# y00njaekim/CMU-11785-IDL-1.58bit-ASR

Measured on AMD Instinct MI355X. Metric: mel-frames/sec (Conformer-S 1.58-bit train step), higher is better.
Workload: dtype fp32; 1 GPU; conformer-s-1.58bit-train-step; global_batch=32, execution=hip-graph, per_gpu_batch=32, frames=1000, d_model=144, blocks=16, d_ff=576, heads=4, vocab=5004, parallelism=dp1, passes=teacher 2-bit + student 1-bit + SP, conv_pointwise=fp32 (reference)

## Files before the change

cmu-11785-idl-1.58bit-asr_amd/csrc/capi.hip:

```cpp
#include <float.h>

#include <algorithm>
#include <vector>

#include "../../include/onebit_hip.h"
#include "ob_launch.h"
#include <stdint.h>

using namespace ob;

namespace {

constexpr int kAbiVersion = 4;

inline hipStream_t as_stream(void* s) { return reinterpret_cast<hipStream_t>(s); }

inline bool aligned4(const void* p) { return (reinterpret_cast<uintptr_t>(p) & 3) == 0; }
inline bool misaligned8(const void* p) { return (reinterpret_cast<uintptr_t>(p) & 7) != 0; }

inline int check_bits(int bits) { return (bits == 1 || bits == 2) ? OB_OK : OB_ERR_BITWIDTH; }

inline int launched() {
  const hipError_t e = hipGetLastError();
  return e == hipSuccess ? OB_OK : OB_ERR_HIP;
// ... 2029 lines not shown
                          void* table, int64_t slot2, int64_t slot1, void* stream) {
  if (rows < 0 || !layernorm_supported(d) || !(p_drop >= 0.0f && p_drop < 1.0f))
    return OB_ERR_SHAPE;
  if (rows > 0 && (!dy || !y1 || !mean2 || !rstd2 || !x || !mean1 || !rstd1 || !dx || !ws))
    return OB_ERR_NULL;
  if (dy2 && p_drop > 0.0f && !rng) return OB_ERR_NULL;
  if (ws_bytes < 2 * layernorm_bwd_workspace(rows, d)) return OB_ERR_WORKSPACE;
  if (!aligned4(dy) || !aligned4(y1) || !aligned4(gres) || !aligned4(x) || !aligned4(dx) ||
      !aligned4(dy2) || !aligned4(g1) || !aligned4(g2) || !aligned4(lens) || ((uintptr_t)ws & 15))
    return OB_ERR_ALIGN;
  if (dy2 && lens && (T < 1 || T > 0x7fffffff || rows % T)) return OB_ERR_SHAPE;
  LnGradScale gsc{dy2, rscale, p_drop, rng, (uint64_t)rng_offset, lens, (int)T};
  LnParamEntry* tab = static_cast<LnParamEntry*>(table);
  const LnDefer f2{tab && slot2 >= 0 ? tab : nullptr, (int)slot2};
  const LnDefer f1{tab && slot1 >= 0 ? tab : nullptr, (int)slot1};
  launch_layernorm_bwd_pair(dy, y1, g2, mean2, rstd2, gres, x, g1, mean1, rstd1, rows, d, dx, dg2,
                            db2, dg1, db1, ws, as_stream(stream), dy2 ? &gsc : nullptr, &f2, &f1);
  return launched();
}

int ob_layernorm_bwd_defer(const float* dy, const float* x, const float* gamma, const float* mean,
                           const float* rstd, int64_t rows, int64_t d, const float* dres,
                           float* dx, float* dgamma, float* dbeta, void* ws, size_t ws_bytes,
                           float* dy2, float rscale, float p_drop, const uint64_t* rng,
                           int64_t rng_offset, const int32_t* lens, int64_t T, void* table,
                           int64_t slot, void* stream) {
  if (table && slot < 0) return OB_ERR_SHAPE;
  if (rows < 0 || !layernorm_supported(d)) return OB_ERR_SHAPE;
  if (rows > 0 && (!dy || !x || !mean || !rstd || !dx)) return OB_ERR_NULL;
  if ((dgamma || dbeta) && !ws) return OB_ERR_NULL;
  if ((dgamma || dbeta) && ws_bytes < layernorm_bwd_workspace(rows, d)) return OB_ERR_WORKSPACE;
  if (!aligned4(dy) || !aligned4(x) || !aligned4(dx) || !aligned4(dres) || !aligned4(dy2) ||
      !aligned4(lens))
    return OB_ERR_ALIGN;
  if (dy2) {
    if (!(p_drop >= 0.0f && p_drop < 1.0f)) return OB_ERR_SHAPE;
    if (lens && (T < 1 || T > 0x7fffffff || rows % T)) return OB_ERR_SHAPE;
    if (p_drop > 0.0f && !rng) return OB_ERR_NULL;
  }
  LnGradScale gs{dy2, rscale, p_drop, rng, (uint64_t)rng_offset,
                 reinterpret_cast<const int*>(lens), (int)T};
  const LnDefer df{static_cast<LnParamEntry*>(table), (int)slot};
  launch_layernorm_bwd(dy, x, gamma, mean, rstd, rows, d, dres, dx, dgamma, dbeta, ws,
                       as_stream(stream), &gs, &df);
  return launched();
}

namespace {
int relattn_check(int64_t Bt, int64_t P, int64_t T, int64_t H, int64_t d, float p_drop) {
  if (Bt < 1 || P < 1 || Bt % P != 0 || H < 1 || !relattn_supported(T, d)) return OB_ERR_SHAPE;
  if (Bt > 65535 || H > 65535 || !(p_drop >= 0.0f && p_drop < 1.0f)) return OB_ERR_SHAPE;
  return OB_OK;
}
}

int ob_relattn_fwd(const float* q, const float* k, const float* v, const float* pos,
                   const float* u, const float* vb, const int32_t* lens, int64_t Bt, int64_t P,
                   int64_t T, int64_t H, int64_t d, float p_drop, const int64_t* rng,
                   int64_t rng_offset, float* saved, float* probs, float* ctx, void* stream) {
  if (int st = relattn_check(Bt, P, T, H, d, p_drop)) return st;
  if (!q || !k || !v || !pos || !u || !vb || !lens || !ctx || (p_drop > 0.0f && !rng))
    return OB_ERR_NULL;
  if (((uintptr_t)saved & 15) || ((uintptr_t)probs & 15)) return OB_ERR_ALIGN;
  launch_relattn_fwd(q, k, v, pos, u, vb, lens, Bt, P, T, H, d, p_drop,
                     reinterpret_cast<const uint64_t*>(rng), (uint64_t)rng_offset, saved, probs,
                     ctx, as_stream(stream));
  return launched();
}

int64_t ob_relattn_saved_elems(int64_t Bt, int64_t T, int64_t H, int64_t d) {
  if (Bt < 1 || H < 1 || !relattn_supported(T, d)) return 0;
  return relattn_saved_elems(Bt, T, H, d);
}

size_t ob_relattn_bwd_workspace(int64_t Bt, int64_t T, int64_t H, int64_t d) {
  if (Bt < 1 || H < 1 || !relattn_supported(T, d)) return 0;
  return align_up(relattn_bwd_workspace(Bt, T, H, d));
}

int ob_relattn_set_bwd_mode(int mode) { return relattn_set_flash(mode); }

int ob_tgemm_set_colloop(int on) { return tgemm_set_colloop(on); }

int64_t ob_relattn_probs_elems(int64_t Bt, int64_t T, int64_t H) {
  if (Bt < 1 || H < 1 || T < 1) return 0;
  return relattn_probs_elems(Bt, T, H);
}

int ob_relattn_bwd(const float* dctx, const float* ctx, const float* q, const float* k,
                   const float* v, const float* pos, const float* u, const float* vb,
                   const int32_t* lens, int64_t Bt, int64_t P, int64_t T, int64_t H, int64_t d,
                   float p_drop, const int64_t* rng, int64_t rng_offset, const float* saved,
                   int64_t saved_elems, float* dq, float* dk, float* dv, float* dpos, float* du,
                   float* dvb, void* ws, size_t ws_bytes, void* stream) {
  if (int st = relattn_check(Bt, P, T, H, d, p_drop)) return st;
  if (!dctx || !ctx || !q || !k || !v || !pos || !u || !vb || !lens || !saved || !dq || !dk ||
      !dv || !dpos || !du || !dvb || !ws)
    return OB_ERR_NULL;
  if (saved_elems != relattn_saved_elems(Bt, T, H, d)) return OB_ERR_SHAPE;
  (void)rng;
  (void)rng_offset;
  if ((uintptr_t)saved & 15) return OB_ERR_ALIGN;
  if (ws_bytes < ob_relattn_bwd_workspace(Bt, T, H, d)) return OB_ERR_WORKSPACE;
  launch_relattn_bwd(dctx, ctx, q, k, v, pos, u, vb, lens, Bt, P, T, H, d, p_drop, saved, dq, dk,
                     dv, dpos, du, dvb, ws, as_stream(stream));
  return launched();
}

int ob_decattn_supported(int64_t Lq, int64_t Lk, int64_t dh) {
  return decattn_supported(Lq, Lk, dh) ? 1 : 0;
}

static int decattn_check(int64_t B, int64_t H, int64_t Lq, int64_t Lk, int64_t dh, int64_t sq,
                         int64_t sk, int64_t sv, float p_drop) {
  if (B < 0 || H < 1 || !decattn_supported(Lq, Lk, dh) || !(p_drop >= 0.0f && p_drop < 1.0f))
    return OB_ERR_SHAPE;
  if (sq < H * dh || sk < H * dh || sv < H * dh) return OB_ERR_SHAPE;
  if (B * H * Lq > INT32_MAX) return OB_ERR_SHAPE;
  return OB_OK;
}

int ob_decattn_fwd(const float* q, int64_t sq, const float* k, int64_t sk, const float* v,
                   int64_t sv, const uint8_t* kmask, int64_t causal, int64_t B, int64_t H,
                   int64_t Lq, int64_t Lk, int64_t dh, float p_drop, const int64_t* rng,
                   int64_t rng_offset, float* probs, float* ctx, void* stream) {
  if (int st = decattn_check(B, H, Lq, Lk, dh, sq, sk, sv, p_drop)) return st;
  if (B > 0 && (!q || !k || !v || !probs || !ctx || (p_drop > 0.0f && !rng))) return OB_ERR_NULL;
  if (!aligned4(q) || !aligned4(k) || !aligned4(v) || !aligned4(probs) ||
      (reinterpret_cast<uintptr_t>(ctx) & 15))
    return OB_ERR_ALIGN;
  launch_decattn_fwd(q, sq, k, sk, v, sv, kmask, causal ? 1 : 0, B, H, Lq, Lk, dh, p_drop,
                     reinterpret_cast<const uint64_t*>(rng), (uint64_t)rng_offset, probs, ctx,
                     as_stream(stream));
  return launched();
}

int ob_decattn_fwd_grouped(const float* q, int64_t sq, const float* k, int64_t sk, const float* v,
                           int64_t sv, const uint8_t* kmask, int64_t causal, int64_t B,
                           int64_t kv_group, int64_t H, int64_t Lq, int64_t Lk, int64_t dh,
                           float* ctx, void* stream) {
  if (kv_group < 1 || B < 0 || (B > 0 && kv_group > INT32_MAX / B)) return OB_ERR_SHAPE;
  if (int st = decattn_check(B * kv_group, H, Lq, Lk, dh, sq, sk, sv, 0.0f)) return st;
  if (B > 0 && (!q || !k || !v || !ctx)) return OB_ERR_NULL;
  if (!aligned4(q) || !aligned4(k) || !aligned4(v) || (reinterpret_cast<uintptr_t>(ctx) & 15))
    return OB_ERR_ALIGN;
  launch_decattn_fwd_grouped(q, sq, k, sk, v, sv, kmask, causal ? 1 : 0, B, kv_group, H, Lq, Lk,
                             dh, ctx, as_stream(stream));
  return launched();
}

int ob_decattn_bwd(const float* dctx, const float* ctx, const float* q, int64_t sq, const float* k,
                   int64_t sk, const float* v, int64_t sv, int64_t B, int64_t H, int64_t Lq, int64_t Lk,
                   int64_t dh, float p_drop, float* probs, float* dq, int64_t gq, float* dk,
                   int64_t gk, float* dv, int64_t gv, void* stream) {
  if (int st = decattn_check(B, H, Lq, Lk, dh, sq, sk, sv, p_drop)) return st;
  if (gq < H * dh || gk < H * dh || gv < H * dh) return OB_ERR_SHAPE;
  if (B > 0 && (!dctx || !ctx || !q || !k || !v || !probs || !dq || !dk || !dv)) return OB_ERR_NULL;
  if (!aligned4(ctx) || !aligned4(dctx) || !aligned4(q) || !aligned4(k) || !aligned4(v) || !aligned4(probs) ||
      !aligned4(dq) || !aligned4(dk) || !aligned4(dv))
    return OB_ERR_ALIGN;
  launch_decattn_bwd(dctx, ctx, q, sq, k, sk, v, sv, B, H, Lq, Lk, dh, p_drop, probs, dq, gq, dk, gk,
                     dv, gv, as_stream(stream));
  return launched();
}

int ob_relattn_dropout_mask(int64_t n, int64_t row_len, float p_drop, const int64_t* rng,
// ... 46 lines not shown
```

cmu-11785-idl-1.58bit-asr_amd/csrc/dgemm.hip:

```cpp
#include <algorithm>
#include <cstdlib>

#include "ob_drop.h"
#include "ob_fp.h"
#include "ob_launch.h"
#include "ob_mma.h"

namespace ob {

namespace {

constexpr size_t kLdsCU = 160 * 1024;

__host__ __device__ inline int dg_kpad(int K, int nch) { return nch > 0 ? 32 * nch : (K + 31) & ~31; }
__host__ __device__ inline size_t dg_lds_bytes(int nt, int kpad) {
  return (size_t)16 * nt * 3 * (kpad + 8) * sizeof(uint16_t);
}

template <int NT, int NCH, int WAVES, bool TRANS, bool RES = false>
__global__ __launch_bounds__(64 * WAVES, 2) void dgemm_kernel(
    const float* __restrict__ A, int64_t M, int K, const float* __restrict__ W, int N, int n_ct,
    int n16, int rgroups, const float* __restrict__ bias, float* __restrict__ C,
    const float* __restrict__ R, DropCfg dc, const uint64_t* __restrict__ rng, uint64_t rng_off) {
  constexpr int kThr = 64 * WAVES, BN = 16 * NT;
  extern __shared__ __attribute__((aligned(16))) char smem[];
  __bf16* bimg = reinterpret_cast<__bf16*>(smem);
  const int kpad = dg_kpad(K, NCH);
  const int stride = kpad + 8;
  const int cpitch = 3 * stride;

  const int L = xcd_logical(blockIdx.x, gridDim.x);
  const int ct = L % n_ct;
  const int rg = L / n_ct;
  const int n0 = ct * BN;
  const int s0 = (int)((int64_t)rg * n16 / rgroups), s1 = (int)((int64_t)(rg + 1) * n16 / rgroups);
  const int lane = threadIdx.x & 63;
  const int wave = threadIdx.x >> 6;
  const int r = lane & 15;
  const int g = lane >> 4;
  const int kg = 8 * g;

  const int kq = kpad >> 2;
  const int units = BN * kq;
  auto unit_cols = [&](int u, int& c, int& k4) {
    if constexpr (TRANS) {
      k4 = u / BN;
      c = u - k4 * BN;
    } else {
      c = u / kq;
      k4 = u - c * kq;
    }
  };
  auto unit_load = [&](int u) -> f32x4 {
    u = u < units ? u : units - 1;
    int c, k4;
    unit_cols(u, c, k4);
    const int n = n0 + c < N ? n0 + c : N - 1;
    const int kk = 4 * k4 < K - 4 ? 4 * k4 : K - 4;
    if constexpr (TRANS) {
      const float* p = W + (int64_t)kk * N + n;
      return f32x4{p[0], p[N], p[2 * N], p[3 * N]};
    } else {
      return *reinterpret_cast<const f32x4*>(W + (int64_t)n * K + kk);
    }
  };
  auto unit_store = [&](int u, f32x4 v) {
    if (u >= units) return;
    int c, k4;
    unit_cols(u, c, k4);
    const bool ok = 4 * k4 < K && n0 + c < N;
    const f32x4 x = ok ? v : f32x4{0.f, 0.f, 0.f, 0.f};
    bf16x4 h, m, l;
    split3x4(x, h, m, l);
    __bf16* col = bimg + c * cpitch + 4 * k4;
    *reinterpret_cast<bf16x4*>(col) = h;
    *reinterpret_cast<bf16x4*>(col + stride) = m;
    *reinterpret_cast<bf16x4*>(col + 2 * stride) = l;
  };
  auto arow_of = [&](int j) {
    const int64_t row = (int64_t)16 * j + r < M ? (int64_t)16 * j + r : M - 1;
    return A + row * (int64_t)K;
  };
  const int j0 = s0 + wave;

// ... 167 lines not shown
    u = u < kUnits ? u : kUnits - 1;
    int c, k4;
    unit_cols(u, c, k4);
    const bool ok = ch * kKc + 4 * k4 < K && c < N;
    const f32x4 x = ok ? v : f32x4{0.f, 0.f, 0.f, 0.f};
    bf16x4 h, m, l;
    split3x4(x, h, m, l);
    __bf16* col = img + buf * kBuf + c * kCpitch + 4 * k4;
    *reinterpret_cast<bf16x4*>(col) = h;
    *reinterpret_cast<bf16x4*>(col + kKcStride) = m;
    *reinterpret_cast<bf16x4*>(col + 2 * kKcStride) = l;
  };
  constexpr int kWin = 4;
  f32x4 abuf[kWin][2];
  auto load_a = [&](int st, f32x4& x0, f32x4& x1) { load8(arow, 32 * st + kg, K, x0, x1); };

  f32x4 wv[kUpt];
#pragma unroll
  for (int i = 0; i < kUpt; ++i) wv[i] = unit_load(0, threadIdx.x + i * kThr);
#pragma unroll
  for (int w = 0; w < kWin; ++w) load_a(w, abuf[w][0], abuf[w][1]);
  __builtin_amdgcn_sched_barrier(0);
#pragma unroll
  for (int i = 0; i < kUpt; ++i) unit_store(0, 0, threadIdx.x + i * kThr, wv[i]);
  __syncthreads();

  f32x4 acc[NT];
#pragma unroll
  for (int t = 0; t < NT; ++t) acc[t] = f32x4{0.f, 0.f, 0.f, 0.f};
  for (int ch0 = 0; ch0 < nck; ch0 += 2) {
#pragma unroll
    for (int cc = 0; cc < 2; ++cc) {
      const int ch = ch0 + cc;
      if (ch >= nck) break;
      const int chn = ch + 1 < nck ? ch + 1 : ch;
#pragma unroll
      for (int i = 0; i < kUpt; ++i) wv[i] = unit_load(chn, threadIdx.x + i * kThr);
      const __bf16* brow = img + cc * kBuf + r * kCpitch + kg;
#pragma unroll
      for (int hs = 0; hs < 2; ++hs) {
        const int st = 2 * ch + hs, slot = 2 * cc + hs;
        const f32x4 x0 = abuf[slot][0], x1 = abuf[slot][1];
        load_a(st + kWin, abuf[slot][0], abuf[slot][1]);
        __builtin_amdgcn_sched_barrier(0);
        constexpr int kG = NT < 3 ? NT : 3;
#pragma unroll
        for (int t0 = 0; t0 < NT; t0 += kG) {
          bf16x8 b[kG][3];
#pragma unroll
          for (int t = 0; t < kG; ++t)
#pragma unroll
            for (int q = 0; q < 3; ++q)
              if (t0 + t < NT)
                b[t][q] = *reinterpret_cast<const bf16x8*>(brow + (t0 + t) * 16 * kCpitch +
                                                            q * kKcStride + 32 * hs);
          __builtin_amdgcn_sched_barrier(0);
          bf16x8 a[3];
          split3x8(x0, x1, a[0], a[1], a[2]);
#pragma unroll
          for (int p = 0; p < 6; ++p)
#pragma unroll
            for (int t = 0; t < kG; ++t)
              if (t0 + t < NT) acc[t0 + t] = mfma_bf16(a[kProdA[p]], b[t][kProdB[p]], acc[t0 + t]);
        }
      }
#pragma unroll
      for (int i = 0; i < kUpt; ++i) unit_store(chn, cc ^ 1, threadIdx.x + i * kThr, wv[i]);
      __syncthreads();
    }
  }
#pragma unroll
  for (int t = 0; t < NT; ++t) {
    const int col = 16 * t + r;
    if (col >= N) continue;
    const float bc = bias ? bias[col] : 0.0f;
#pragma unroll
    for (int reg = 0; reg < 4; ++reg) {
      const int64_t orow = m0 + 4 * g + reg;
      if (orow < M) C[orow * N + col] = acc[t][reg] + bc;
    }
  }
}

struct DgCfg {
  int nt, waves;
};

DgCfg pick_cfg(int64_t N, int64_t K) {
  const int kpad = dg_kpad((int)K, 0);
  const bool k_special = kpad == 160 || kpad == 288;
  static const int cands[] = {9, 6, 3, 2, 1};
  for (int pass = 0; pass < 2; ++pass)
    for (int nt : cands) {
      if (pass == 0 && N % (16 * nt) != 0) continue;
      if (16 * nt > ((N + 15) & ~int64_t(15))) continue;
      const bool inst = kpad == 160 ? (nt == 9 || nt == 6 || nt == 3)
                        : kpad == 288 ? (nt == 3 || nt == 2 || nt == 1)
                                      : (nt == 3 || nt == 1);
      if (!inst && k_special) continue;
      if (!k_special && !(nt == 3 || nt == 1)) continue;
      const size_t lds = dg_lds_bytes(nt, kpad);
      int waves = lds <= kLdsCU / 2 ? 4 : lds <= kLdsCU ? 8 : 0;
      if (waves) return DgCfg{nt, waves};
    }
  return DgCfg{0, 0};
}

}

static bool dense_kc_shape(int64_t K, int64_t N) {
  return N >= 4 && N <= 144 && N % 4 == 0 && K >= 4 && K % 4 == 0 && K <= (1 << 20) &&
         pick_cfg(N, K).nt == 0;
}

bool dense_gemm_supported(int64_t K, int64_t N) {
  return (K >= 4 && N >= 4 && K % 4 == 0 && N % 4 == 0 && K <= (1 << 20) && N <= (1 << 20) &&
          pick_cfg(N, K).nt > 0) ||
         dense_kc_shape(K, N);
}

bool launch_dense_gemm(const float* A, int64_t M, int64_t K, const float* W, int trans,
                       const float* bias, int64_t N, float* C, hipStream_t s,
                       const DenseEpi* epi) {
  if (!dense_gemm_supported(K, N)) return false;
  if (M == 0) return true;
  if (dense_kc_shape(K, N)) {
    if (epi && epi->R) return false;
    constexpr int kW = 8;
    const dim3 grid((unsigned)ceil_div(M, 16 * kW));
    const size_t lds = dgkc_lds_bytes(9);
    if (trans)
      hipLaunchKernelGGL((dgemm_kc_kernel<9, kW, true>), grid, dim3(64 * kW), lds, s, A, M, (int)K,
                         W, (int)N, bias, C);
    else
      hipLaunchKernelGGL((dgemm_kc_kernel<9, kW, false>), grid, dim3(64 * kW), lds, s, A, M,
                         (int)K, W, (int)N, bias, C);
    return true;
  }
  const DgCfg cfg = pick_cfg(N, K);
  const int kpad = dg_kpad((int)K, 0);
  const size_t lds = dg_lds_bytes(cfg.nt, kpad);
  const int n_ct = (int)ceil_div(N, 16 * cfg.nt);
  const int n16 = (int)ceil_div(M, 16);
  const int per_cu = (int)std::min<size_t>(kLdsCU / lds, (size_t)(8 / cfg.waves));
  int rgroups = 256 * per_cu / n_ct;
  rgroups = std::min<int64_t>(rgroups, ceil_div(n16, cfg.waves));
  if (rgroups < 1) rgroups = 1;
  const dim3 grid((unsigned)(rgroups * n_ct));
  const int nch = kpad == 160 ? 5 : kpad == 288 ? 9 : 0;
  const float* R = epi ? epi->R : nullptr;
  const DropCfg dc = make_drop(R ? epi->p_drop : 0.0f);
  const uint64_t* rng = R ? epi->rng : nullptr;
  const uint64_t rng_off = R ? epi->rng_off : 0;
#define OB_DG(NT, NCH, WV)                                                                       \
  if (cfg.nt == NT && nch == NCH && cfg.waves == WV) {                                           \
    if (trans)                                                                                   \
      hipLaunchKernelGGL((dgemm_kernel<NT, NCH, WV, true>), grid, dim3(64 * WV), lds, s, A, M,    \
                         (int)K, W, (int)N, n_ct, n16, rgroups, bias, C, nullptr, dc,    \
                         nullptr, 0);                                                            \
    else                                                                                         \
      hipLaunchKernelGGL((dgemm_kernel<NT, NCH, WV, false>), grid, dim3(64 * WV), lds, s, A, M,   \
                         (int)K, W, (int)N, n_ct, n16, rgroups, bias, C, nullptr, dc,    \
                         nullptr, 0);                                                            \
    return true;                                                                                 \
  }
#define OB_DG2(NT, NCH) OB_DG(NT, NCH, 4) OB_DG(NT, NCH, 8)
  if (R && !trans && cfg.nt == 9 && nch == 5) {
#define OB_DGR(WV)                                                                               \
    if (cfg.waves == WV) {                                                                       \
      hipLaunchKernelGGL((dgemm_kernel<9, 5, WV, false, true>), grid, dim3(64 * WV), lds, s, A,   \
                         M, (int)K, W, (int)N, n_ct, n16, rgroups, bias, C, R, dc, rng,         \
                         rng_off);                                                               \
      return true;                                                                               \
    }
    OB_DGR(4)
    OB_DGR(8)
#undef OB_DGR
  }
  if (R) {
    DenseEpi none{nullptr, 0.0f, nullptr, 0};
    if (!launch_dense_gemm(A, M, K, W, trans, bias, N, C, s, &none)) return false;
    launch_residual_drop_fwd(R, C, M, N, 1.0f, epi->p_drop, rng, rng_off, nullptr, 0, C, s);
    return true;
  }
  OB_DG2(9, 5)
  OB_DG2(6, 5)
  OB_DG2(3, 5)
  OB_DG2(3, 9)
  OB_DG2(2, 9)
  OB_DG2(1, 9)
  OB_DG2(3, 0)
  OB_DG2(1, 0)
#undef OB_DG2
#undef OB_DG
  return false;
}

}
```

cmu-11785-idl-1.58bit-asr_amd/csrc/ob_launch.h:

```cpp
#pragma once

#include <hip/hip_runtime.h>
#include <stddef.h>
#include <stdint.h>

#include "../../include/onebit_hip.h"

namespace ob {

inline int64_t ceil_div(int64_t a, int64_t b) { return (a + b - 1) / b; }

void launch_quant_pack(const float* W, const float* alpha, int alpha_raw, int bits,
                       const int* bits_dev, int64_t N, int64_t K, uint32_t* codes,
                       uint32_t* codes_t, hipStream_t s);
int64_t quant_pack_item_blocks(int64_t N, int64_t K);
int64_t quant_pack_item_blocks16(int64_t N, int64_t K);
void launch_quant_pack_group(const ob_pack_item* items_dev, int n_items, int64_t total_blocks,
                             hipStream_t s);
void launch_quant_dequant(const float* W, const float* alpha, int alpha_raw, int bits, int64_t n,
                          float* W_hat, hipStream_t s);

int64_t ste_reduce_blocks(int64_t total);
void launch_ste_reduce(const float* part, int chunks, int64_t nk, const float* part_db,
                       int64_t n_db, const float* W, const float* alpha, int alpha_raw, int bits,
// ... 119 lines not shown
  const float* W;
  const float* alpha;
  int alpha_raw;
  int bits;
  const int* bits_dev;
  const int* pass_bits;
  float* apart;
};
void launch_dw_partial(const float* dY, const float* X, int64_t M, int64_t N, int64_t K,
                       const DwPlan& p, float* part, float* part_db, uint32_t* ticket,
                       hipStream_t s, const DwAlpha* al = nullptr);
void launch_dw_partial_group(const float* const* dY, int G, const float* X, int64_t M,
                             int64_t N, int64_t K, const DwPlan& p, float* const* part,
                             float* const* part_db, const DwAlpha* al, hipStream_t s);
void launch_dw_finish(const float* part, int chunks, int64_t nk, const float* part_db,
                      int64_t n_db, const float* W, const float* alpha, int alpha_raw,
                      const float* apart, int n_apart, float* dW, float* db, float* dalpha,
                      hipStream_t s);

struct DwFinish {
  const float* part;
  int chunks;
  int64_t nk;
  const float* part_db;
  int64_t n_db;
  const float* W;
  const float* alpha;
  int alpha_raw;
  const float* apart;
  int n_apart;
  float* dW;
  float* db;
  float* dalpha;
};
constexpr int kMaxDwGroup = 3;
void launch_dw_finish_group(const DwFinish* a, int n, hipStream_t s);

struct DwFinishEntry {
  DwFinish f;
  int64_t start;
};
int64_t dw_finish_blocks(const DwFinish& a);
void launch_dw_table_entry(DwFinishEntry* table, int slot, const DwFinishEntry& ent, hipStream_t s);
void launch_dw_finish_table(const DwFinishEntry* table, int n, int64_t total_blocks, hipStream_t s);
void launch_dw_partial_group_defer(const float* const* dY, int G, const float* X, int64_t M,
                                   int64_t N, int64_t K, const DwPlan& p, float* const* part,
                                   float* const* part_db, const DwAlpha* al,
                                   DwFinishEntry* table, int slot, const DwFinishEntry* ent,
                                   hipStream_t s);

struct DwgDesc {
  const float* dY;
  const float* X;
  const float* W;
  const float* alpha;
  const int* pass_bits;
  float* dW;
  float* db;
  float* dalpha;
  int64_t work0;
  int N, K, Mp, P, alpha_raw, bits;
  int spp;
  int tiles_k;
  int tiles;
  int tile0;
};
constexpr int kDwgTile = 144;
int dwg_blocks(int64_t total_steps);
size_t dwg_slot_bytes();
void launch_dw_grouped(const DwgDesc* host_descs, int G, int64_t total_steps, int blocks,
                       DwgDesc* table, float* slots, float* talpha, uint32_t* tickets,
                       int total_tiles, hipStream_t s);

bool dense_gemm_supported(int64_t K, int64_t N);
struct DenseEpi {
  const float* R;
  float p_drop;
  const uint64_t* rng;
  uint64_t rng_off;
};
bool launch_dense_gemm(const float* A, int64_t M, int64_t K, const float* W, int trans,
                       const float* bias, int64_t N, float* C, hipStream_t s,
                       const DenseEpi* epi = nullptr);

bool ternary_gemm_i8_supported(int64_t K, int64_t N);
void launch_silu_monotone_check(uint32_t lo, uint32_t hi, uint32_t* bad, hipStream_t s);
size_t act_absmax_workspace(int P);
void launch_act_absmax(const float* X, int P, int64_t n_per_pass, float* amax, void* ws,
                       hipStream_t s);
void launch_act_dequant(const float* X, int P, int64_t n_per_pass, const float* amax, float* Xd,
                        hipStream_t s);
bool launch_ternary_gemm_i8(const float* A, int P, int64_t M, int64_t K, const uint32_t* codes,
                            const uint32_t* codes1, const int* pass_bits, int64_t N,
                            const float* alpha, int alpha_raw, const float* amax,
                            const float* bias, float* C, hipStream_t s);

void launch_ctc_greedy(const float* logits, const int64_t* lens, int64_t B, int64_t T, int64_t V,
                       int blank, int* ids, int* out, int* out_len, hipStream_t s);

struct CtcBeamLm {
  const void* table;
  int64_t slots;
  int max_probe, order;
  double unk_logp;
  int bos, eos;
  double lm_weight, ins_bonus;
  double *ctc, *lm, *total;
};
size_t ctc_beam_workspace(int64_t B, int64_t T, int64_t V, int beam, int top_k);
void launch_ctc_beam(const float* logits, const int64_t* lens, int64_t B, int64_t T, int64_t V,
                     int blank, int beam, int top_k, int stages, void* ws, int* hyp, int* hyp_len,
                     int* n_hyp, double* score, int nbest, const CtcBeamLm* lm, hipStream_t s);

bool seq_logprob_supported(int64_t d, int64_t V);
size_t seq_logprob_workspace(int64_t R, int64_t d, int64_t V);
void launch_seq_logprob(const float* hidden, int64_t R, int64_t d, const float* weight,
                        const float* bias, int64_t V, const int* target, void* ws, float* lp,
                        hipStream_t s);
void launch_rescore_prepare(const int* hyp, const int* hyp_len, const int* n_hyp, int64_t B,
                            int64_t N, int64_t T, int64_t Lc, int bos, int eos, int pad,
                            int64_t* tgt_inp, int* target, uint8_t* tgt_pad, uint8_t* ok,
                            hipStream_t s);
void launch_rescore_select(const float* lp, const int* hyp, const int* hyp_len, const int* n_hyp,
                           const double* ctc, const double* lm, const uint8_t* ok, int64_t B,
                           int64_t N, int64_t T, int64_t Lc, double ctc_weight, double lm_weight,
                           int* out, int* out_len, int* best_k, double* att, double* total,
                           uint8_t* rescored, hipStream_t s);

constexpr int kSeqTopkMaxBanned = 8;
struct AttdecState {
  double* score;
  int* len;
  uint8_t* fin;
  int64_t* tok;
  uint8_t* skip;
};
bool attdec_supported(int64_t N, int64_t d, int64_t H, int64_t Lk, int64_t L);
void launch_decattn_step(const float* qkv, int64_t sq, float* cache, const int* anc,
                         const uint8_t* skip, int64_t R, int64_t H, int64_t dh, int64_t L,
                         int64_t t, float* ctx, hipStream_t s);
size_t seq_topk_workspace(int64_t R, int64_t d, int64_t V, int64_t K);
void launch_seq_topk(const float* hidden, int64_t R, int64_t d, const float* weight,
                     const float* bias, int64_t V, const int* banned, int n_banned,
                     const uint8_t* skip, int64_t K, void* ws, double* lse, float* topv,
                     int* topi, hipStream_t s);
void launch_attdec_init(const uint8_t* kmask, int64_t B, int64_t N, int64_t Lk, int64_t L, int bos,
                        const AttdecState& st, int* anc, hipStream_t s);
constexpr int kStepBeam = 0, kStepJoint = 1, kStepFused = 2;
void launch_attdec_step(int mode, const double* lse, const float* topv, const int* topi,
                        const double* cpsi, double w, const double* lmsc, double lw, int64_t B,
                        int64_t N, int64_t K, int64_t L, int64_t t, int eos, int pad,
                        const double* norm, const int* anc_in, int* anc_out,
                        const AttdecState& st, double* att, double* ctc, double* lm, int* link,
                        int* tr_parent, int* tr_token, double* tr_score, hipStream_t s);
void launch_attdec_finalize(const int* tr_parent, const int* tr_token, const AttdecState& st,
                            int64_t B, int64_t N, int64_t L, int eos, int* hyp, int* hyp_len,
                            int* n_hyp, double* score, uint8_t* finished, hipStream_t s);

bool ctc_prefix_supported(int64_t N, int64_t K, int64_t Tp);
size_t ctc_prefix_workspace(int64_t B, int64_t N, int64_t K, int64_t Tp);
void launch_ctc_frame_lse(const float* logits, const int64_t* lens, int64_t B, int64_t Tp,
                          int64_t V, double* flse, hipStream_t s);
void launch_ctc_prefix_step(const float* logits, const double* flse, const int64_t* lens,
                            const int* topi, const int64_t* tok, const int* len, const int* link,
                            const uint8_t* skip, int64_t B, int64_t N, int64_t K, int64_t Tp,
                            int64_t V, int blank, int eos, const double* st_in, double* st_out,
// ... 202 lines not shown
```

cmu-11785-idl-1.58bit-asr_amd/onebit_asr/_lib.py:

```python
from __future__ import annotations

import ctypes
import os
from pathlib import Path

import torch

LIB_NAME = "libonebit_hip.so"
LIB_PATH = Path(os.environ.get("ONEBIT_HIP_LIB") or Path(__file__).with_name(LIB_NAME))

OB_OK = 0
OB_ERR_SHAPE = -2
OB_ERR_BITWIDTH = -3

_c_f = ctypes.c_void_p
_i64 = ctypes.c_int64
_int = ctypes.c_int
_sz = ctypes.c_size_t
_f32 = ctypes.c_float
_f64 = ctypes.c_double

SIGNATURES = {
    "ob_abi_version": (_int, []),
    "ob_source_digest": (ctypes.c_char_p, []),
# ... 171 lines not shown
    "ob_nbest_edit_distance": (_int, [_c_f, _c_f, _c_f, _c_f, _c_f, _i64, _i64, _i64, _i64, _c_f,
                                      _sz, _c_f, _c_f, _c_f, _c_f]),
    "ob_mbr_select": (_int, [_c_f, _c_f, _c_f, _c_f, _c_f, _f64, _i64, _i64, _i64, _c_f, _c_f,
                             _c_f, _c_f, _c_f, _c_f]),
    "ob_fbank_num_frames": (_i64, [_i64]),
    "ob_frontend_table_floats": (_i64, [_int]),
    "ob_frontend_table_fill": (_int, [_c_f, _int]),
    "ob_frontend_fwd": (_int, [_c_f, _i64, _c_f, _i64, _i64, _c_f, _int, _c_f, _c_f, _c_f, _int,
                               _int, _int, _int, _c_f, _i64, _c_f, _c_f]),
    "ob_layernorm_fwd": (_int, [_c_f, _c_f, _c_f, _i64, _i64, _f32, _c_f, _c_f, _c_f, _c_f]),
    "ob_layernorm_fwd_pair": (_int, [_c_f, _c_f, _c_f, _c_f, _c_f, _i64, _i64, _f32, _f32, _c_f,
                                     _c_f, _c_f, _c_f, _c_f, _c_f, _c_f]),
    "ob_layernorm_fwd_amax_workspace": (_sz, [_i64]),
    "ob_layernorm_fwd_amax": (_int, [_c_f, _c_f, _c_f, _i64, _i64, _f32, _c_f, _c_f, _c_f, _i64,
                                     _c_f, _c_f, _sz, _c_f]),
    "ob_layernorm_fwd_i8": (_int, [_c_f, _c_f, _c_f, _i64, _i64, _f32, _i64, _c_f, _c_f, _c_f,
                                   _sz, _c_f]),
    "ob_layernorm_bwd_defer": (
        _int, [_c_f, _c_f, _c_f, _c_f, _c_f, _i64, _i64, _c_f, _c_f, _c_f, _c_f, _c_f, _sz, _c_f,
               _f32, _f32, _c_f, _i64, _c_f, _i64, _c_f, _i64, _c_f]),
    "ob_layernorm_bwd_pair_workspace": (_sz, [_i64, _i64]),
    "ob_layernorm_bwd_pair": (
        _int, [_c_f, _c_f, _c_f, _c_f, _c_f, _c_f, _c_f, _c_f, _c_f, _c_f, _i64, _i64, _c_f, _c_f,
               _c_f, _c_f, _c_f, _c_f, _sz, _c_f, _f32, _f32, _c_f, _i64, _c_f, _i64, _c_f, _i64,
               _i64, _c_f]),
    "ob_ln_param_entry_bytes": (_sz, []),
    "ob_ln_param_table": (_int, [_c_f, _i64, _i64, _c_f]),
    "ob_dw_finish_entry_bytes": (_sz, []),
    "ob_bitlinear_bwd_dw_passes_defer": (
        _int, [_c_f, _c_f, _i64, _i64, _i64, _i64, _c_f, _c_f, _int, _c_f, _c_f, _c_f, _c_f, _c_f,
               _sz, _c_f, _i64, _i64, _c_f, _c_f]),
    "ob_bitlinear_bwd_dw_passes_group_defer": (
        _int, [_i64, _c_f, _c_f, _i64, _i64, _i64, _i64, _c_f, _c_f, _int, _c_f, _c_f, _c_f, _c_f,
               _c_f, _sz, _c_f, _i64, _i64, _c_f, _c_f]),
    "ob_dw_finish_table": (_int, [_c_f, _i64, _i64, _c_f]),
    "ob_dw_grouped_supported": (_int, [_i64, _i64]),
    "ob_dw_grouped_workspace": (_sz, [_c_f, _i64]),
    "ob_dw_grouped_tickets": (_sz, [_c_f, _i64]),
    "ob_dw_grouped": (_int, [_c_f, _i64, _c_f, _sz, _c_f, _sz, _c_f]),
    "ob_dense_dw_defer": (_int, [_c_f, _c_f, _i64, _i64, _i64, _c_f, _c_f, _c_f, _sz, _c_f, _i64,
                                 _i64, _c_f, _c_f]),
    "ob_layernorm_bwd_workspace": (_sz, [_i64, _i64]),
    "ob_layernorm_bwd": (
        _int, [_c_f, _c_f, _c_f, _c_f, _c_f, _i64, _i64, _c_f, _c_f, _c_f, _c_f, _sz, _c_f]),
    "ob_layernorm_bwd_res": (
        _int, [_c_f, _c_f, _c_f, _c_f, _c_f, _i64, _i64, _c_f, _c_f, _c_f, _c_f, _c_f, _sz, _c_f]),
    "ob_layernorm_bwd_ex": (
        _int, [_c_f, _c_f, _c_f, _c_f, _c_f, _i64, _i64, _c_f, _c_f, _c_f, _c_f, _c_f, _sz, _c_f,
               _f32, _f32, _c_f, _i64, _c_f, _i64, _c_f]),
    "ob_act_absmax_workspace": (_sz, [_i64]),
    "ob_act_absmax": (_int, [_c_f, _i64, _i64, _c_f, _c_f, _sz, _c_f]),
    "ob_act_dequant_i8": (_int, [_c_f, _i64, _i64, _c_f, _c_f, _c_f]),
    "ob_bitlinear_fwd_i8": (
        _int, [_c_f, _i64, _i64, _i64, _c_f, _c_f, _c_f, _c_f, _int, _c_f, _c_f, _i64, _c_f, _c_f]),
    "ob_bitlinear_fwd_i8_epi": (
        _int, [_c_f, _i64, _i64, _i64, _c_f, _c_f, _c_f, _c_f, _int, _c_f, _c_f, _i64, _int, _c_f,
               _f32, _c_f, _i64, _c_f, _c_f, _c_f]),
    "ob_bitlinear_fwd_passes_group": (
        _int, [_i64, _c_f, _i64, _i64, _i64, _c_f, _c_f, _c_f, _c_f, _int, _c_f, _i64, _c_f, _c_f]),
    "ob_bitlinear_fwd_i8q": (
        _int, [_c_f, _i64, _i64, _i64, _c_f, _c_f, _c_f, _c_f, _int, _c_f, _c_f, _i64, _int, _c_f,
               _f32, _c_f, _i64, _c_f, _c_f, _c_f]),
    "ob_bitlinear_bwd_dx_passes": (
        _int, [_c_f, _i64, _i64, _i64, _c_f, _c_f, _c_f, _c_f, _int, _i64, _c_f, _c_f]),
    "ob_bitlinear_bwd_dw_passes_workspace": (_sz, [_i64, _i64, _i64, _i64]),
    "ob_bitlinear_bwd_dw_passes": (
        _int, [_c_f, _c_f, _i64, _i64, _i64, _i64, _c_f, _c_f, _int, _c_f, _c_f, _c_f, _c_f, _c_f,
               _sz, _c_f]),
    "ob_bitlinear_bwd_dw_passes_group_workspace": (_sz, [_i64, _i64, _i64, _i64, _i64]),
    "ob_bitlinear_bwd_dw_passes_group": (
        _int, [_i64, _c_f, _c_f, _i64, _i64, _i64, _i64, _c_f, _c_f, _int, _c_f, _c_f, _c_f, _c_f,
               _c_f, _sz, _c_f]),
    "ob_relattn_fwd": (
        _int, [_c_f, _c_f, _c_f, _c_f, _c_f, _c_f, _c_f, _i64, _i64, _i64, _i64, _i64, _f32, _c_f,
               _i64, _c_f, _c_f, _c_f, _c_f]),
    "ob_relattn_saved_elems": (_i64, [_i64, _i64, _i64, _i64]),
    "ob_relattn_probs_elems": (_i64, [_i64, _i64, _i64]),
    "ob_relattn_bwd_workspace": (_sz, [_i64, _i64, _i64, _i64]),
    "ob_relattn_bwd": (
        _int, [_c_f, _c_f, _c_f, _c_f, _c_f, _c_f, _c_f, _c_f, _c_f, _i64, _i64, _i64, _i64, _i64,
               _f32, _c_f, _i64, _c_f, _i64, _c_f, _c_f, _c_f, _c_f, _c_f, _c_f, _c_f, _sz, _c_f]),
    "ob_relattn_set_bwd_mode": (_int, [_int]),
    "ob_tgemm_set_colloop": (_int, [_int]),
    "ob_relattn_dropout_mask": (_int, [_i64, _i64, _f32, _c_f, _i64, _c_f, _c_f]),
    "ob_embedding_bwd": (_int, [_c_f, _i64, _c_f, _i64, _i64, _i64, _c_f, _c_f]),
    "ob_adamw_plan": (_i64, [_c_f, _i64, _c_f]),
    "ob_adamw_workspace": (_sz, [_i64]),
    "ob_adamw_clip_step": (
        _int, [_c_f, _i64, _c_f, _i64, _c_f, _c_f, _f32, _f64, _f64, _f64, _f64, _f64, _c_f, _c_f,
               _sz, _c_f]),
}

ABI_VERSION = 4

_lib = None


class OneBitHipError(RuntimeError):
    pass


def load() -> ctypes.CDLL:
    global _lib
    if _lib is not None:
        return _lib
    if not LIB_PATH.is_file():
        raise OneBitHipError(
            f"{LIB_PATH} is missing: build it with `make -C cmu-11785-idl-1.58bit-asr_amd/csrc` "
            "(or __graft_entry__.build()); there is no CPU fallback for the BitLinear path"
        )
    lib = ctypes.CDLL(str(LIB_PATH))
    for name, (res, args) in SIGNATURES.items():
        fn = getattr(lib, name)
        fn.restype = res
        fn.argtypes = args
    if lib.ob_abi_version() != ABI_VERSION:
        raise OneBitHipError(f"ABI mismatch: library {lib.ob_abi_version()} != {ABI_VERSION}")
    check_digest(lib)
    _lib = lib
    return lib


def check_digest(lib, expected: str | None = None) -> None:
    if expected is None:
        if os.environ.get("ONEBIT_HIP_LIB"):
            return
        if not _sources_present():
            import warnings

            warnings.warn(f"{LIB_PATH.name}: no csrc/ sources beside it; build digest not checked")
            return
        expected = source_digest()
    got = lib.ob_source_digest().decode()
    if got != expected:
        raise OneBitHipError(
            f"{LIB_PATH.name} was built from other sources (digest {got[:12]} != {expected[:12]} "
            "of csrc/ and include/): rebuild with `make -C cmu-11785-idl-1.58bit-asr_amd/csrc`")


def _sources_present() -> bool:
    csrc = Path(__file__).resolve().parents[1] / "csrc"
    return csrc.is_dir() and any(csrc.glob("*.hip"))


def ptr_array(ptrs):
    return (ctypes.c_void_p * len(ptrs))(*[p or None for p in ptrs])


def check(status: int, what: str) -> None:
    if status == OB_OK:
        return
    msg = load().ob_status_string(status).decode()
    if status == OB_ERR_BITWIDTH:
        raise ValueError("bitwidth must be one of {1,2,32}")
    raise OneBitHipError(f"{what}: {msg} (status {status})")


def ptr(t: "torch.Tensor | None") -> int | None:
    return None if t is None else t.data_ptr()


def source_digest() -> str:
    from ._digest import source_digest as _sd

    return _sd()

# ... 4 lines not shown
```

include/onebit_hip.h:

```cpp
#ifndef ONEBIT_HIP_H_
#define ONEBIT_HIP_H_

#include <stddef.h>
#include <stdint.h>

#ifdef __cplusplus
extern "C" {
#endif

#define OB_API __attribute__((visibility("default")))

enum {
  OB_OK = 0,
  OB_ERR_NULL = -1,
  OB_ERR_SHAPE = -2,
  OB_ERR_BITWIDTH = -3,
  OB_ERR_WORKSPACE = -4,
  OB_ERR_ALIGN = -5,
  OB_ERR_HIP = -6
};

OB_API int ob_abi_version(void);
OB_API const char* ob_source_digest(void);
OB_API const char* ob_status_string(int status);
// ... 435 lines not shown
                              const int32_t* tlen, int64_t B, int64_t Tp, int64_t V, int64_t S,
                              int blank, int stage, void* ws, size_t ws_bytes, int32_t* path,
                              int32_t* span, double* tok_score, double* score, void* stream);

OB_API int ob_edit_supported(int64_t La, int64_t Lb);
OB_API size_t ob_edit_distance_workspace(int64_t P, int64_t La, int64_t Lb);
OB_API int ob_edit_distance(const int32_t* a, const int32_t* a_len, const int32_t* b,
                            const int32_t* b_len, int64_t P, int64_t La, int64_t Lb, void* ws,
                            size_t ws_bytes, int32_t* dist, int32_t* ops, void* stream);
OB_API size_t ob_nbest_edit_distance_workspace(int64_t B, int64_t N, int64_t T, int64_t S);
OB_API int ob_nbest_edit_distance(const int32_t* hyp, const int32_t* hyp_len,
                                  const int32_t* n_hyp, const int32_t* ref,
                                  const int32_t* ref_len, int64_t B, int64_t N, int64_t T,
                                  int64_t S, void* ws, size_t ws_bytes, int32_t* dref,
                                  int32_t* ops_ref, int32_t* dpair, void* stream);
OB_API int ob_mbr_select(const int32_t* dpair, const int32_t* hyp, const int32_t* hyp_len,
                         const int32_t* n_hyp, const double* score, double scale, int64_t B,
                         int64_t N, int64_t T, int32_t* out, int32_t* out_len, int32_t* best_k,
                         double* risk, double* post, void* stream);

OB_API int64_t ob_fbank_num_frames(int64_t n_samples);
OB_API int64_t ob_frontend_table_floats(int n_mels);
OB_API int ob_frontend_table_fill(float* host_table, int n_mels);
OB_API int ob_frontend_fwd(const float* wave, int64_t wave_stride, const int64_t* wave_lens,
                           int64_t B, int64_t n_max, const float* table, int n_mels,
                           const float* cmvn_mean, const float* cmvn_std,
                           const int32_t* mask_starts, int n_fmask, int fmask_w, int n_tmask,
                           int tmask_w, float* feats, int64_t T, int64_t* feat_lens,
                           void* stream);

OB_API int ob_bitlinear_fwd_swish_drop(const float* X, int64_t P, int64_t M, int64_t K,
                                       const uint32_t* codes2, const uint32_t* codes1,
                                       const int32_t* pass_bits, const float* alpha,
                                       int alpha_raw, const float* bias, int64_t N, float p_drop,
                                       const uint64_t* rng, int64_t rng_offset, float* Y_pre,
                                       float* Y_act, void* stream);
OB_API int ob_bitlinear_fwd_residual(const float* X, int64_t P, int64_t M, int64_t K,
                                     const uint32_t* codes2, const uint32_t* codes1,
                                     const int32_t* pass_bits, const float* alpha, int alpha_raw,
                                     const float* bias, int64_t N, const float* R, float rscale,
                                     float p_drop, const uint64_t* rng, int64_t rng_offset,
                                     const int32_t* lens, int64_t T, float* Y, void* stream);
OB_API int ob_bitlinear_fwd_residual_ln(
    const float* X, int64_t P, int64_t M, int64_t K, const uint32_t* codes2,
    const uint32_t* codes1, const int32_t* pass_bits, const float* alpha, int alpha_raw,
    const float* bias, int64_t N, const float* R, float rscale, float p_drop, const uint64_t* rng,
    int64_t rng_offset, const int32_t* lens, int64_t T, float* Y, int nln, const float* ln_w0,
    const float* ln_b0, float eps0, float* ln_y0, float* ln_mean0, float* ln_rstd0,
    const float* ln_w1, const float* ln_b1, float eps1, float* ln_y1, float* ln_mean1,
    float* ln_rstd1, void* stream);
OB_API int ob_bitlinear_bwd_dx_swish_drop(const float* dY, int64_t P, int64_t M, int64_t N,
                                          const uint32_t* codes2_t, const uint32_t* codes1_t,
                                          const int32_t* pass_bits, const float* alpha,
                                          int alpha_raw, int64_t K, const float* pre,
                                          float p_drop, const uint64_t* rng, int64_t rng_offset,
                                          float* dPre, void* stream);
OB_API int ob_drop_scale_bwd(const float* dOut, int64_t rows, int64_t N, float rscale,
                             float p_drop, const uint64_t* rng, int64_t rng_offset,
                             const int32_t* lens, int64_t T, float* dY, void* stream);

OB_API int ob_residual_drop_fwd(const float* R, const float* Y, int64_t rows, int64_t N,
                                float rscale, float p_drop, const uint64_t* rng,
                                int64_t rng_offset, const int32_t* lens, int64_t T, float* out,
                                void* stream);

OB_API int ob_bias_relu_fwd(float* y, const float* bias, int64_t B, int64_t C, int64_t hw,
                            void* stream);
OB_API size_t ob_relu_bias_bwd_workspace(int64_t B, int64_t C);
OB_API int ob_relu_bias_bwd(const float* g, const float* y, int64_t B, int64_t C, int64_t hw,
                            float* gout, float* dbias, void* ws, size_t ws_bytes, void* stream);
OB_API size_t ob_colsum_workspace(int64_t N);
OB_API int ob_colsum(const float* x, int64_t rows, int64_t N, float* out, void* ws,
                     size_t ws_bytes, void* stream);

OB_API int ob_silu_fast_monotone_check(uint32_t lo_bits, uint32_t hi_bits, uint32_t* bad,
                                       void* stream);
OB_API int ob_dense_supported(int64_t K, int64_t N);
OB_API int ob_dense_gemm(const float* X, int64_t M, int64_t K, const float* W, int w_trans,
                         const float* bias, int64_t N, float* Y, void* stream);
OB_API int ob_dense_gemm_residual_drop(const float* X, int64_t M, int64_t K, const float* W,
                                       const float* bias, int64_t N, const float* R,
                                       float p_drop, const int64_t* rng, int64_t rng_offset,
                                       float* Y, void* stream);
OB_API size_t ob_dense_dw_workspace(int64_t M, int64_t N, int64_t K);
OB_API int ob_dense_dw(const float* dY, const float* X, int64_t M, int64_t N, int64_t K,
                       float* dW, float* db, void* ws, size_t ws_bytes, void* stream);
OB_API int ob_dense_dw_defer(const float* dY, const float* X, int64_t M, int64_t N, int64_t K,
                             float* dW, float* db, void* ws, size_t ws_bytes, void* table,
                             int64_t slot, int64_t start, int64_t* n_blocks, void* stream);

OB_API size_t ob_convmod_workspace(int64_t P, int64_t Bt, int64_t T, int64_t C, int64_t K);
OB_API int ob_convmod_fwd(const float* u, const float* w_dw, const float* b_dw,
                          const float* gamma, const float* beta, int64_t P, int64_t Bt,
                          int64_t T, int64_t C, int64_t K, float eps, float* z, float* g,
                          float* stats, float* v, void* ws, size_t ws_bytes, void* stream);
OB_API int ob_convmod_bwd(const float* dv, const float* u, const float* z, const float* g,
                          const float* stats, const float* w_dw, const float* gamma,
                          const float* beta, int64_t P, int64_t Bt, int64_t T, int64_t C,
                          int64_t K, float* du, float* dw_dw, float* db_dw, float* dgamma,
                          float* dbeta, void* ws, size_t ws_bytes, void* stream);
OB_API int ob_convmod_bwd_defer(const float* dv, const float* u, const float* z, const float* g,
                                const float* stats, const float* w_dw, const float* gamma,
                                const float* beta, int64_t P, int64_t Bt, int64_t T, int64_t C,
                                int64_t K, float* du, float* dw_dw, float* db_dw, float* dgamma,
                                float* dbeta, void* ws, size_t ws_bytes, void* table, int64_t slot,
                                int64_t* deferred, void* stream);
OB_API size_t ob_cm_wgrad_entry_bytes(void);
OB_API int ob_cm_wgrad_table(const void* table, int64_t n, int64_t nmax, void* stream);

OB_API size_t ob_subsample_image_bytes(int64_t C);
OB_API int ob_subsample_pack(const float* W2, int64_t C, void* img, void* stream);
OB_API int ob_subsample_fwd(const float* X, int64_t B, int64_t T, int64_t F, int64_t C,
                            const float* W0, const float* b0, const void* img,
                            const float* b2, float* Y1, float* Y2, void* stream);
OB_API size_t ob_subsample_bwd_workspace(int64_t B, int64_t T, int64_t F, int64_t C);
OB_API int ob_subsample_bwd(const float* X, const float* W0, const float* b0, const float* Y1,
                            const float* Y2, const float* dY2, int64_t B, int64_t T, int64_t F,
                            int64_t C, const void* img,
                            float* dW0, float* db0, float* dW2, float* db2, void* ws,
                            size_t ws_bytes, void* stream);

#ifdef __cplusplus
}
#endif

#endif
```

Measured before the change: 1.420 million mel-frames/s.

## Add register-resident row-streaming dense GEMM kernel for K=160 shapes

Adds a single-wave dense GEMM kernel for K padded to 160 (nch==5). It keeps the split-bf16 weight fragments for a 48-column group in registers and streams 16-row tiles of A through a register prefetch window, interleaving MFMA with loads via sched barriers. It replaces the LDS-staged dgemm path for residual/dropout epilogues and for small problems, and is enabled by default behind a runtime toggle. The intent is to avoid LDS staging and syncthreads overhead, at the cost of high register pressure and lower occupancy.

```diff
diff --git a/cmu-11785-idl-1.58bit-asr_amd/csrc/capi.hip b/cmu-11785-idl-1.58bit-asr_amd/csrc/capi.hip
--- a/cmu-11785-idl-1.58bit-asr_amd/csrc/capi.hip
+++ b/cmu-11785-idl-1.58bit-asr_amd/csrc/capi.hip
@@ -2135,6 +2135,8 @@
 
 int ob_tgemm_set_colloop(int on) { return tgemm_set_colloop(on); }
 
+int ob_dense_set_rowstream(int on) { return dense_set_rowstream(on); }
+
 int64_t ob_relattn_probs_elems(int64_t Bt, int64_t T, int64_t H) {
   if (Bt < 1 || H < 1 || T < 1) return 0;
   return relattn_probs_elems(Bt, T, H);
diff --git a/cmu-11785-idl-1.58bit-asr_amd/csrc/dgemm.hip b/cmu-11785-idl-1.58bit-asr_amd/csrc/dgemm.hip
--- a/cmu-11785-idl-1.58bit-asr_amd/csrc/dgemm.hip
+++ b/cmu-11785-idl-1.58bit-asr_amd/csrc/dgemm.hip
@@ -1,5 +1,7 @@
 #include <algorithm>
+#include <atomic>
 #include <cstdlib>
+#include <type_traits>
 
 #include "ob_drop.h"
 #include "ob_fp.h"
@@ -333,6 +335,165 @@
   }
 }
 
+template <int NT, int NCH, int WIN, bool TRANS, bool RES = false>
+__global__ __launch_bounds__(64) void dgemm_rowstream_kernel(
+    const float* __restrict__ A, int64_t M, int K, const float* __restrict__ W, int N, int n_cg,
+    int n16, int rshares, const float* __restrict__ bias, float* __restrict__ C,
+    const float* __restrict__ R, DropCfg dc, const uint64_t* __restrict__ rng, uint64_t rng_off) {
+  constexpr int BN = 16 * NT;
+  static_assert(WIN >= 2 && WIN <= NCH, "chunks in flight");
+  const int L = xcd_logical(blockIdx.x, gridDim.x);
+  const int cg = L % n_cg;
+  const int rs = L / n_cg;
+  const int n0 = cg * BN;
+  const int s0 = (int)((int64_t)rs * n16 / rshares), s1 = (int)((int64_t)(rs + 1) * n16 / rshares);
+  if (s0 >= s1) return;
+  const int lane = threadIdx.x & 63;
+  const int r = lane & 15;
+  const int g = lane >> 4;
+  const int kg = 8 * g;
+
+  auto arow_of = [&](int j) {
+    const int64_t row = (int64_t)16 * j + r < M ? (int64_t)16 * j + r : M - 1;
+    return A + row * (int64_t)K;
+  };
+  f32x4 buf[NCH][2];
+  {
+    const float* a0 = arow_of(s0);
+#pragma unroll
+    for (int c = 0; c < WIN; ++c) load8(a0, 32 * c + kg, K, buf[c][0], buf[c][1]);
+  }
+
+  bf16x8 b[NT][NCH][3];
+#pragma unroll
+  for (int t = 0; t < NT; ++t) {
+    const int col = n0 + 16 * t + r;
+    const bool cok = col < N;
+    const int cn = cok ? col : N - 1;
+#pragma unroll
+    for (int c = 0; c < NCH; ++c) {
+      const int k = 32 * c + kg;
+      f32x4 x0, x1;
+      if constexpr (TRANS) {
+#pragma unroll
+        for (int j = 0; j < 8; ++j) {
+          const int kk = k + j < K - 1 ? k + j : K - 1;
+          const float v = W[(int64_t)kk * N + cn];
+          if (j < 4) x0[j] = v;
+          else x1[j - 4] = v;
+        }
+      } else {
+        load8(W + (int64_t)cn * K, k, K, x0, x1);
+      }
+      const f32x4 zero{0.f, 0.f, 0.f, 0.f};
+      x0 = (cok && k < K) ? x0 : zero;
+      x1 = (cok && k + 4 < K) ? x1 : zero;
+      split3x8(x0, x1, b[t][c][0], b[t][c][1], b[t][c][2]);
+    }
+  }
+
+  const uint32_t dkey = (RES && dc.on) ? drop_key(rng[0], rng[1] + rng_off) : 0u;
+  float bcol[NT];
+#pragma unroll
+  for (int t = 0; t < NT; ++t) {
+    const int col = n0 + 16 * t + r;
+    bcol[t] = (bias && col < N) ? bias[col] : 0.0f;
+  }
+  const bool cols_in = n0 + BN <= N;
+
+  auto epilogue = [&](auto full, int64_t m0, const f32x4 (&acc)[NT]) {
+#pragma unroll
+    for (int t = 0; t < NT; ++t) {
+      const int col = n0 + 16 * t + r;
+      if (!full.value && col >= N) continue;
+      float rv[4];
+      if constexpr (RES) {
+#pragma unroll
+        for (int reg = 0; reg < 4; ++reg)
+          rv[reg] = R[min(m0 + 4 * g + reg, M - 1) * N + col];
+      }
+#pragma unroll
+      for (int reg = 0; reg < 4; ++reg) {
+        const int64_t orow = m0 + 4 * g + reg;
+        if (!full.value && orow >= M) continue;
+        const int64_t i = orow * N + col;
+        const float y = acc[t][reg] + bcol[t];
+        if constexpr (RES) {
+          const float v = dc.on ? nc_mul(y, drop_keep(dkey, (uint64_t)i, dc.thresh) ? dc.scale : 0.0f) : y;
+          C[i] = nc_add(rv[reg], v);
+        } else {
+          C[i] = y;
+        }
+      }
+    }
+  };
+
+  uint32_t a[2][3][4];
+  auto frag = [&](int par, int q) {
+    return __builtin_bit_cast(bf16x8, u32x4{a[par][q][0], a[par][q][1], a[par][q][2], a[par][q][3]});
+  };
+#pragma unroll
+  for (int q = 0; q < 4; ++q)
+    split2(buf[0][q >> 1][2 * (q & 1)], buf[0][q >> 1][2 * (q & 1) + 1], a[0][0][q], a[0][1][q],
+           a[0][2][q]);
+  constexpr int kMf = 6 * NT, kMfQ = (kMf + 3) / 4;
+  for (int j = s0; j < s1; ++j) {
+    const int64_t m0 = (int64_t)16 * j;
+    const float* arow = arow_of(j);
+    const float* anext = arow_of(j + 1 < s1 ? j + 1 : j);
+    f32x4 acc[NT];
+#pragma unroll
+    for (int t = 0; t < NT; ++t) acc[t] = f32x4{0.f, 0.f, 0.f, 0.f};
+
+#pragma unroll
+    for (int c = 0; c < NCH; ++c) {
+      const int cn = (c + 1) % NCH;
+      const int par = c & 1;
+      const bf16x8 af[3] = {frag(par, 0), frag(par, 1), frag(par, 2)};
+#pragma unroll
+      for (int q = 0; q < 4; ++q) {
+        __builtin_amdgcn_sched_barrier(0);
+        split2(buf[cn][q >> 1][2 * (q & 1)], buf[cn][q >> 1][2 * (q & 1) + 1], a[par ^ 1][0][q],
+               a[par ^ 1][1][q], a[par ^ 1][2][q]);
+        if (q == 0) {
+          if (c + WIN < NCH)
+            load8(arow, 32 * (c + WIN) + kg, K, buf[c + WIN][0], buf[c + WIN][1]);
+          else
+            load8(anext, 32 * (c + WIN - NCH) + kg, K, buf[c + WIN - NCH][0],
+                  buf[c + WIN - NCH][1]);
+        }
+#pragma unroll
+        for (int i = q * kMfQ; i < (q + 1) * kMfQ && i < kMf; ++i) {
+          const int pp = i / NT, t = i % NT;
+          acc[t] = mfma_bf16(af[kProdA[pp]], b[t][c][kProdB[pp]], acc[t]);
+        }
+#pragma unroll
+        for (int i = 0; i < kMfQ; ++i) {
+          __builtin_amdgcn_sched_group_barrier(0x008, 1, 0);
+          __builtin_amdgcn_sched_group_barrier(0x002, 3, 0);
+        }
+      }
+    }
+    __builtin_amdgcn_sched_barrier(0);
+    if constexpr (NCH & 1) {
+#pragma unroll
+      for (int q = 0; q < 3; ++q)
+#pragma unroll
+        for (int w = 0; w < 4; ++w) a[0][q][w] = a[1][q][w];
+    }
+    if (cols_in && m0 + 16 <= M) epilogue(std::true_type{}, m0, acc);
+    else epilogue(std::false_type{}, m0, acc);
+  }
+}
+
+constexpr int64_t kRsMaxN = 432;
+constexpr int kRsNT = 3;
+constexpr int kRsWin = 5;
+constexpr int kRsWaves = 1024;
+constexpr int kRsMaxSub2 = 5;
+
+std::atomic<int> g_rowstream{1};
+
 struct DgCfg {
   int nt, waves;
 };
@@ -362,6 +523,12 @@
 static bool dense_kc_shape(int64_t K, int64_t N) {
   return N >= 4 && N <= 144 && N % 4 == 0 && K >= 4 && K % 4 == 0 && K <= (1 << 20) &&
          pick_cfg(N, K).nt == 0;
+}
+
+int dense_set_rowstream(int on) {
+  const int prev = g_rowstream.load(std::memory_order_relaxed);
+  if (on == 0 || on == 1) g_rowstream.store(on, std::memory_order_relaxed);
+  return prev;
 }
 
 bool dense_gemm_supported(int64_t K, int64_t N) {
@@ -403,6 +570,22 @@
   const DropCfg dc = make_drop(R ? epi->p_drop : 0.0f);
   const uint64_t* rng = R ? epi->rng : nullptr;
   const uint64_t rng_off = R ? epi->rng_off : 0;
+  if (nch == 5 && N <= kRsMaxN && g_rowstream.load(std::memory_order_relaxed) == 1) {
+    const int n_cg = (int)ceil_div(N, 16 * kRsNT);
+    const bool few = 2 * (int64_t)n16 * n_cg <= (int64_t)kRsMaxSub2 * kRsWaves;
+    if (R ? !trans : few) {
+      const int rshares = std::max(1, std::min(n16, kRsWaves / n_cg));
+      const dim3 rgrid((unsigned)(rshares * n_cg));
+#define OB_RS(TR, RS)                                                                            \
+  hipLaunchKernelGGL((dgemm_rowstream_kernel<kRsNT, 5, kRsWin, TR, RS>), rgrid, dim3(64), 0, s,  \
+                     A, M, (int)K, W, (int)N, n_cg, n16, rshares, bias, C, R, dc, rng, rng_off)
+      if (R) OB_RS(false, true);
+      else if (trans) OB_RS(true, false);
+      else OB_RS(false, false);
+#undef OB_RS
+      return true;
+    }
+  }
 #define OB_DG(NT, NCH, WV)                                                                       \
   if (cfg.nt == NT && nch == NCH && cfg.waves == WV) {                                           \
     if (trans)                                                                                   \
diff --git a/cmu-11785-idl-1.58bit-asr_amd/csrc/ob_launch.h b/cmu-11785-idl-1.58bit-asr_amd/csrc/ob_launch.h
--- a/cmu-11785-idl-1.58bit-asr_amd/csrc/ob_launch.h
+++ b/cmu-11785-idl-1.58bit-asr_amd/csrc/ob_launch.h
@@ -225,6 +225,7 @@
 bool launch_dense_gemm(const float* A, int64_t M, int64_t K, const float* W, int trans,
                        const float* bias, int64_t N, float* C, hipStream_t s,
                        const DenseEpi* epi = nullptr);
+int dense_set_rowstream(int on);
 
 bool ternary_gemm_i8_supported(int64_t K, int64_t N);
 void launch_silu_monotone_check(uint32_t lo, uint32_t hi, uint32_t* bad, hipStream_t s);
diff --git a/cmu-11785-idl-1.58bit-asr_amd/onebit_asr/_lib.py b/cmu-11785-idl-1.58bit-asr_amd/onebit_asr/_lib.py
--- a/cmu-11785-idl-1.58bit-asr_amd/onebit_asr/_lib.py
+++ b/cmu-11785-idl-1.58bit-asr_amd/onebit_asr/_lib.py
@@ -277,6 +277,7 @@
                _f32, _c_f, _i64, _c_f, _i64, _c_f, _c_f, _c_f, _c_f, _c_f, _c_f, _c_f, _sz, _c_f]),
     "ob_relattn_set_bwd_mode": (_int, [_int]),
     "ob_tgemm_set_colloop": (_int, [_int]),
+    "ob_dense_set_rowstream": (_int, [_int]),
     "ob_relattn_dropout_mask": (_int, [_i64, _i64, _f32, _c_f, _i64, _c_f, _c_f]),
     "ob_embedding_bwd": (_int, [_c_f, _i64, _c_f, _i64, _i64, _i64, _c_f, _c_f]),
     "ob_adamw_plan": (_i64, [_c_f, _i64, _c_f]),
diff --git a/include/onebit_hip.h b/include/onebit_hip.h
--- a/include/onebit_hip.h
+++ b/include/onebit_hip.h
@@ -541,6 +541,7 @@
                                        const float* bias, int64_t N, const float* R,
                                        float p_drop, const int64_t* rng, int64_t rng_offset,
                                        float* Y, void* stream);
+OB_API int ob_dense_set_rowstream(int on);
 OB_API size_t ob_dense_dw_workspace(int64_t M, int64_t N, int64_t K);
 OB_API int ob_dense_dw(const float* dY, const float* X, int64_t M, int64_t N, int64_t K,
                        float* dW, float* db, void* ws, size_t ws_bytes, void* stream);
```

Result: no change. 1.424 million mel-frames/s, median of 6 (+0.3%).
